# juno181/Ex4DGS

Measured on AMD Instinct MI355X. Metric: fwd+bwd ms/frame @1M Gaussians 1352x1014; achieved HBM GB/s vs peak, lower is better.
Workload: dtype f32; 1 GPU; cfg3: 1.0M static+dynamic (K=35), 1352x1014; P=1000000, HW=1370928, sh_degree=3, step=GaussianRasterizer forward + backward on a resident frame, parallelism=frame-sharded x1

## Files before the change

### ex4dgs_amd/csrc/ex4d_api.hip

```cpp
#include "ex4d_internal.h"
#include <atomic>
#include <cstdarg>
#include <cstdio>
#include <cstdlib>
#include <cstring>
#include <mutex>

namespace {

std::atomic<bool> g_prof_on{false};
std::atomic<int> g_bwd_variant{4};
std::atomic<int> g_tile_ids{0};
std::atomic<int> g_tile_rows{1};
std::atomic<int> g_depth_msd{3};
struct DepthSortWatch {
    std::mutex mu;
    uint32_t *word = nullptr;
    bool tried = false;
    std::atomic<int> hold{0}, backoff{64}, trips{0};
    uint32_t *get()
    {
        std::lock_guard<std::mutex> lock(mu);
        if (!tried) {
            tried = true;
            if (hipHostMalloc((void **)&word, 64, hipHostMallocPortable) != hipSuccess) { (void)hipGetLastError(); word = nullptr; }
            else memset(word, 0, 64);
        }
        return word;
    }
    void reset()
    {
        std::lock_guard<std::mutex> lock(mu);
        hold.store(0); backoff.store(64); trips.store(0);
        if (word) __atomic_store_n(word, 0u, __ATOMIC_RELAXED);
// ... 429 lines not shown
    const float *shs, const float *colors_precomp, const float *scales, const float *rotations,
    const float *cov3D_precomp, const float *viewmatrix, const float *projmatrix, const float *campos,
    const float *subpixel_offset, const float *out_depth, const float *out_acc,
    const void *geom_buffer, const void *binning_buffer, const void *img_buffer,
    const float *dL_dout_color, const float *dL_dout_depth, const float *dL_dout_flow, const float *dL_dout_acc,
    float *dL_dmeans2D, float *dL_dcolors, float *dL_dopacity, float *dL_dmeans3D, float *dL_dcov3D, float *dL_dsh,
    float *dL_dscales, float *dL_drotations, float *dL_ddir, void *bwd_scratch, void *stream_)
{
    g_err[0] = 0;
    hipStream_t stream = (hipStream_t)stream_;
    if (!prm) return fail(EX4D_ERR_ARG, "null params");
    const int P = prm->P, W = prm->W, H = prm->H;
    if (P <= 0 || W <= 0 || H <= 0) return fail(EX4D_ERR_ARG, "P, W, H must be positive (P == 0 is handled by the caller)");
    if (!geom_buffer || !binning_buffer || !img_buffer || !bwd_scratch) return fail(EX4D_ERR_ARG, "null state buffer");
    if ((size_t)P * 64 > 0xFFFFFFFFull) return fail(EX4D_ERR_ARG, "more than 2^26 Gaussians: the accumulator rows are addressed with 32-bit byte offsets");
    if (!dL_dmeans2D || !dL_dopacity || !dL_dmeans3D || !dL_dscales || !dL_drotations || !dL_ddir || (prm->M > 0 && !dL_dsh && !(gsplit.rest[0] || gsplit.rest[1])))
        return fail(EX4D_ERR_ARG, "null gradient output");
    GeomState g = carve_geom((void *)geom_buffer, P, nullptr, nullptr);
    BinState b = carve_binning((void *)binning_buffer, (uint32_t)num_rendered, W, H, nullptr, nullptr);
    ImgState im = carve_img((void *)img_buffer, W, H, nullptr, nullptr);
    float *acc16 = (float *)bwd_scratch;

    const int variant = g_bwd_variant.load(std::memory_order_relaxed);
    g_prof.begin(1, stream);
    HIP_TRY(ex4d_launch_zero(acc16, (size_t)P * 16 * sizeof(float), stream));
    MARK(1, "zero_accumulators");
    if (num_rendered > 0)
        STAGE(ex4d_launch_composite_bwd(*prm, im.ranges, b.point_list, subpixel_offset, background, g.records,
                                        out_depth, out_acc, im.final_T, im.n_contrib,
                                        dL_dout_color, dL_dout_depth, dL_dout_flow, dL_dout_acc, acc16, b.qlist, b.qcount, variant, stream), prm, stream);
    MARK(1, "composite_bwd");
    const float *cov3D_ptr = cov3D_precomp;
    STAGE(ex4d_launch_preprocess_bwd(*prm, means3D, radii, shs, scales, rotations, cov3D_ptr, viewmatrix, projmatrix, campos, g, acc16,
                                     dL_dmeans2D, dL_dcolors, dL_dopacity, dL_dmeans3D, dL_dcov3D, dL_dsh, dL_dscales, dL_drotations, dL_ddir,
                                     split, gsplit, stream), prm, stream);
    MARK(1, "preprocess_bwd");
    return EX4D_OK;
}

static const ShSplit kNoSplit = { { nullptr, nullptr }, { nullptr, nullptr }, 0 };
static const ShSplitGrad kNoSplitGrad = { { nullptr, nullptr }, { nullptr, nullptr }, 0 };

int ex4d_forward(
    const Ex4dParams *prm,
    const float *background, const float *means3D, const float *dir3D, const float *shs, const float *colors_precomp,
    const float *opacities, const float *scales, const float *rotations, const float *cov3D_precomp,
    const float *viewmatrix, const float *projmatrix, const float *campos, const float *subpixel_offset,
    ex4d_alloc_fn geom_alloc, void *geom_user, ex4d_alloc_fn binning_alloc, void *binning_user,
    ex4d_alloc_fn img_alloc, void *img_user,
    float *out_color, int32_t *radii, float *out_depth, float *out_acc, float *out_flow, int32_t *out_idx,
    void *stream_, int32_t *num_rendered)
{
    return forward_impl(prm, kNoSplit, background, means3D, dir3D, shs, colors_precomp, opacities, scales, rotations, cov3D_precomp,
                        viewmatrix, projmatrix, campos, subpixel_offset, geom_alloc, geom_user, binning_alloc, binning_user,
                        img_alloc, img_user, out_color, radii, out_depth, out_acc, out_flow, out_idx, stream_, num_rendered);
}

static bool split_ok(const Ex4dParams *prm, const float *const dc[2], const float *const rest[2], int n_static)
// ... 49 lines not shown
    float *dL_dmeans2D, float *dL_dcolors, float *dL_dopacity, float *dL_dmeans3D, float *dL_dcov3D, const Ex4dSplitSHGrad *dL_dsh,
    float *dL_dscales, float *dL_drotations, float *dL_ddir, void *bwd_scratch, void *stream_)
{
    g_err[0] = 0;
    if (!shs || !dL_dsh || !split_ok(prm, shs->dc, shs->rest, shs->n_static) || dL_dsh->n_static != shs->n_static ||
        !split_ok(prm, (const float *const *)dL_dsh->dc, (const float *const *)dL_dsh->rest, dL_dsh->n_static))
        return fail(EX4D_ERR_ARG, "split SH: null tensor, n_static outside [0, P] or mismatching gradient split");
    if (prm->M != 16) return fail(EX4D_ERR_ARG, "split SH needs M == 16 (dc [n,1,3] + rest [n,15,3])");
    const ShSplit sp = { { shs->dc[0], shs->dc[1] }, { shs->rest[0], shs->rest[1] }, shs->n_static };
    const ShSplitGrad gsp = { { dL_dsh->dc[0], dL_dsh->dc[1] }, { dL_dsh->rest[0], dL_dsh->rest[1] }, dL_dsh->n_static };
    return backward_impl(prm, sp, gsp, num_rendered, background, means3D, radii, nullptr, nullptr, scales, rotations,
                         cov3D_precomp, viewmatrix, projmatrix, campos, subpixel_offset, out_depth, out_acc, geom_buffer, binning_buffer,
                         img_buffer, dL_dout_color, dL_dout_depth, dL_dout_flow, dL_dout_acc, dL_dmeans2D, dL_dcolors, dL_dopacity,
                         dL_dmeans3D, dL_dcov3D, nullptr, dL_dscales, dL_drotations, dL_ddir, bwd_scratch, stream_);
}

int ex4d_set_option(const char *name, int value)
{
    if (name && !strcmp(name, "composite_bwd_variant") && (value == 4 || value == 8)) { g_bwd_variant.store(value); return EX4D_OK; }
    if (name && !strcmp(name, "composite_fwd_asm") && (value == 0 || value == 1)) { ex4d_set_fwd_asm(value); return EX4D_OK; }
    if (name && !strcmp(name, "binning_tile_ids") && (value == 0 || value == 1)) { g_tile_ids.store(value); return EX4D_OK; }
    if (name && !strcmp(name, "composite_clamp_always") && (value == 0 || value == 1)) { ex4d_set_clamp_always(value); return EX4D_OK; }
    if (name && !strcmp(name, "composite_bwd_pairs") && (value == 0 || value == 1)) { ex4d_set_bwd_pairs(value); return EX4D_OK; }
    if (name && !strcmp(name, "tile_sort_rows") && (value == 0 || value == 1)) { g_tile_rows.store(value); return EX4D_OK; }
    if (name && !strcmp(name, "rank_lds_atomics") && value >= -1 && value <= 1) { ex4d_set_rank_lds(value); return EX4D_OK; }
    if (name && !strcmp(name, "rows_probe")) { ex4d_set_rows_probe(value); return EX4D_OK; }
    if (name && !strcmp(name, "preprocess_sh_predicate") && (value == 0 || value == 1)) { ex4d_set_preprocess_tune(value); return EX4D_OK; }
    if (name && !strcmp(name, "geom_debug_arrays") && (value == 0 || value == 1)) { g_geom_debug.store(value); return EX4D_OK; }
    if (name && !strcmp(name, "preprocess_fast_path") && (value == 0 || value == 1)) { ex4d_set_preprocess_fast(value); return EX4D_OK; }
    if (name && !strcmp(name, "depth_sort_msd") && value >= 0 && value <= 3) { g_depth_msd.store(value); g_depth_watch.reset(); return EX4D_OK; }
    if (name && !strcmp(name, "depth_sort_local_cap") && value >= 0 && value <= 8192) { g_depth_local_cap.store(value); return EX4D_OK; }
    if (name && !strcmp(name, "readback_side_stream") && (value == 0 || value == 1)) { g_readback_side.store(value); return EX4D_OK; }
    if (name && !strcmp(name, "depth_sort_msd_bits") && (value == 0 || value == EX4D_DLS_MSD_BITS - 1 || value == EX4D_DLS_MSD_BITS)) { g_depth_msd_bits.store(value); return EX4D_OK; }
    if (name && !strcmp(name, "depth_sort_local_threads") && (value == 0 || value == 256 || value == 512)) { g_depth_local_threads.store(value); return EX4D_OK; }
    return fail(EX4D_ERR_ARG, "unknown option or value out of range");
}

int ex4d_debug_bwd_stats(unsigned long long *out8, int reset) { return ex4d_bwd_stats(out8, 8, reset) == hipSuccess ? EX4D_OK : EX4D_ERR_HIP; }
int ex4d_debug_rows_prof(unsigned long long *out8, int reset) { return ex4d_rows_prof(out8, reset) == hipSuccess ? EX4D_OK : EX4D_ERR_HIP; }
int ex4d_debug_bwd_stats16(unsigned long long *out16, int reset) { return ex4d_bwd_stats(out16, 16, reset) == hipSuccess ? EX4D_OK : EX4D_ERR_HIP; }

int ex4d_get_option(const char *name)
{
    if (name && !strcmp(name, "composite_bwd_variant")) return g_bwd_variant.load();
    if (name && !strcmp(name, "composite_fwd_asm")) return ex4d_get_fwd_asm();
    if (name && !strcmp(name, "binning_tile_ids")) return g_tile_ids.load();
    if (name && !strcmp(name, "composite_clamp_always")) return ex4d_get_clamp_always();
    if (name && !strcmp(name, "composite_bwd_pairs")) return ex4d_get_bwd_pairs();
    if (name && !strcmp(name, "tile_sort_rows")) return g_tile_rows.load();
    if (name && !strcmp(name, "rank_lds_atomics")) return ex4d_get_rank_lds();
    if (name && !strcmp(name, "rank_lds_atomics_in_use")) return ex4d_rank_lds_in_use();
    if (name && !strcmp(name, "preprocess_sh_predicate")) return ex4d_get_preprocess_tune();
    if (name && !strcmp(name, "geom_debug_arrays")) return g_geom_debug.load();
    if (name && !strcmp(name, "preprocess_fast_path")) return ex4d_get_preprocess_fast();
    if (name && !strcmp(name, "depth_sort_msd")) return g_depth_msd.load();
    if (name && !strcmp(name, "depth_sort_hold")) return g_depth_watch.hold.load();
    if (name && !strcmp(name, "depth_sort_trips")) return g_depth_watch.trips.load();
    if (name && !strcmp(name, "depth_sort_local_cap")) return g_depth_local_cap.load();
    if (name && !strcmp(name, "readback_side_stream")) return g_readback_side.load();
    if (name && !strcmp(name, "depth_sort_msd_bits")) return g_depth_msd_bits.load();
    if (name && !strcmp(name, "depth_sort_local_threads")) return g_depth_local_threads.load();
    return -1;
}

void ex4d_profile_enable(int on) { g_prof_on.store(on != 0); }

int ex4d_profile_read(int which, float *ms, const char **names, int max_stages)
{
    std::lock_guard<std::mutex> lock(g_prof.mu);
    if (which < 0 || which > 1 || !g_prof.created) return 0;
    const int n = g_prof.n[which] < max_stages ? g_prof.n[which] : max_stages;
// ... 23 lines not shown
```

### ex4dgs_amd/csrc/ex4d_composite.hip

```cpp
#include "ex4d_internal.h"
#include <hip/amd_detail/amd_hip_unsafe_atomics.h>
#include <atomic>

namespace {

__device__ __forceinline__ void wave_lds_sync()
{
    __builtin_amdgcn_fence(__ATOMIC_RELEASE, "wavefront");
    __builtin_amdgcn_wave_barrier();
    __builtin_amdgcn_fence(__ATOMIC_ACQUIRE, "wavefront");
}

typedef unsigned long long lanemask;
#define LANES(cmp) __builtin_amdgcn_ballot_w64(cmp)
__device__ __forceinline__ float select_f(lanemask m, float if_set, float if_clear)
{
    float r;
    asm("s_nop 1\n\tv_cndmask_b32_e64 %0, %1, %2, %3" : "=v"(r) : "v"(if_clear), "v"(if_set), "s"(m));
    return r;
}
__device__ __forceinline__ int select_i(lanemask m, int if_set, int if_clear)
{
    int r;
    asm("s_nop 1\n\tv_cndmask_b32_e64 %0, %1, %2, %3" : "=v"(r) : "v"(if_clear), "v"(if_set), "s"(m));
// ... 757 lines not shown
    }
    wave_lds_sync();
    {
        float v[13];
        const float Se = S2.x, So = S2.y, Ye = Y2.x, Yo = Y2.y;
        v[0] = dxe * Se + dxo * So;
        v[1] = Ye + Yo;
        v[3] = (dxe * dxe) * Se + (dxo * dxo) * So;
        v[4] = dxe * Ye + dxo * Yo;
        v[0] *= w; v[1] *= w; v[3] *= w; v[4] *= w;
        v[5] = w * (M5.x + M5.y);
        v[2] = v2.x + v2.y; v[6] = Se + So; v[7] = c7.x + c7.y; v[8] = c8.x + c8.y; v[9] = c9.x + c9.y;
        v[10] = c10.x + c10.y; v[11] = c11.x + c11.y; v[12] = c12.x + c12.y;
        {
            const float m0 = v[0], m1 = v[1];
            v[0] = (2.f * ap) * m0 + bp * m1;
            v[1] = (2.f * cp) * m1 + bp * m0;
            v[2] *= flagf;
        }
        bwd_batch_finish<NOLAST>(L, nvalid, acc16, v, __float_as_uint(g1.w), n, g);
    }
}

template <int WPB, bool STATS>
__global__ __launch_bounds__(64 * WPB, 4) void composite_bwd_scan_kernel(
    int W, int H, int gx, int num_tiles,
    const uint2 *__restrict__ ranges, const uint32_t *__restrict__ point_list,
    const float *__restrict__ subpixel_offset, const float *__restrict__ bg,
    const float4 *__restrict__ records,
    const float *__restrict__ depth_acc, const float *__restrict__ weight_acc, float min_depth,
    const float *__restrict__ final_Ts, const uint32_t *__restrict__ n_contrib,
    const float *__restrict__ dL_dpixels, const float *__restrict__ dL_ddepths,
    const float *__restrict__ dL_dflows, const float *__restrict__ dL_daccs,
    float *__restrict__ acc16, const uint32_t *__restrict__ qlist, const uint32_t *__restrict__ qcount, int pairs_on)
{
    constexpr int RING = BWD_RING;
    __shared__ BwdLdsT<RING> lds[WPB];
    int tile, quad;
    tile_of_block(num_tiles, tile, quad);
    if (tile >= num_tiles) return;
    const int wave = (WPB == 4) ? (threadIdx.x >> 6) : 0, lane = threadIdx.x & 63;
    BwdLdsT<RING> &L = lds[wave];
    const PixelGeom p = pixel_of_lane(tile, quad, gx, W, H, subpixel_offset);
    const uint2 range = ranges[tile];
    const size_t HW = (size_t)H * W;
    const uint32_t last_contributor = p.inside ? n_contrib[p.pix_id] : 0u;
    const uint32_t deepest = wave_max_u32(last_contributor);
    if (deepest == 0) return;
    const uint32_t min_last = wave_min_u32(last_contributor);

    const float T_final = p.inside ? final_Ts[p.pix_id] : 0.f;
    const float acc = p.inside ? weight_acc[p.pix_id] : 0.f;
    const float final_depth = p.inside ? depth_acc[p.pix_id] : 0.f;
    float gdepth = 0.f, gflow0 = 0.f, gflow1 = 0.f, gflow2 = 0.f, gacc = 0.f, gp0 = 0.f, gp1 = 0.f, gp2 = 0.f;
    if (p.inside) {
        if (dL_ddepths) gdepth = dL_ddepths[p.pix_id];
        if (dL_dpixels) { gp0 = dL_dpixels[p.pix_id]; gp1 = dL_dpixels[HW + p.pix_id]; gp2 = dL_dpixels[2 * HW + p.pix_id]; }
        if (acc > 0.0f) {
            gdepth /= acc;
            if (dL_dflows) { gflow0 = dL_dflows[p.pix_id] / acc; gflow1 = dL_dflows[HW + p.pix_id] / acc; gflow2 = dL_dflows[2 * HW + p.pix_id] / acc; }
// ... 100 lines not shown

hipError_t ex4d_launch_composite_fwd(const Ex4dParams &prm, const uint2 *ranges, const uint32_t *point_list,
    const float *subpixel_offset, const float4 *records, const float *bg, float *final_T, uint32_t *n_contrib,
    float *out_color, float *out_depth, float *out_acc, float *out_flow, int32_t *out_idx, uint32_t *qlist, uint32_t *qcount,
    bool has_flow, hipStream_t stream)
{
    const int gx = (prm.W + EX4D_TILE - 1) / EX4D_TILE, gy = (prm.H + EX4D_TILE - 1) / EX4D_TILE;
    const int T = gx * gy;
    const int slots = 8 * ((T + 7) / 8);
#define FWD_LAUNCH(FLOW) hipLaunchKernelGGL((composite_fwd_kernel<FLOW, ASM>), dim3(4 * slots), dim3(64), 0, stream, \
        prm.W, prm.H, gx, T, ranges, point_list, subpixel_offset, records, bg, \
        prm.max_depth, final_T, n_contrib, out_color, out_depth, out_acc, out_flow, out_idx, qlist, qcount, g_alpha_clamp_always.load(std::memory_order_relaxed))
    if (has_flow) { constexpr bool ASM = false; FWD_LAUNCH(true); }
    else if (g_fwd_asm.load(std::memory_order_relaxed)) { constexpr bool ASM = true; FWD_LAUNCH(false); }
    else { constexpr bool ASM = false; FWD_LAUNCH(false); }
#undef FWD_LAUNCH
    return hipGetLastError();
}

hipError_t ex4d_launch_composite_bwd(const Ex4dParams &prm, const uint2 *ranges, const uint32_t *point_list,
    const float *subpixel_offset, const float *bg, const float4 *records, const float *out_depth, const float *out_acc,
    const float *final_T, const uint32_t *n_contrib, const float *dL_dpix, const float *dL_ddepth,
    const float *dL_dflow, const float *dL_dacc, float *acc16, const uint32_t *qlist, const uint32_t *qcount,
    int variant, hipStream_t stream)
{
    const int gx = (prm.W + EX4D_TILE - 1) / EX4D_TILE, gy = (prm.H + EX4D_TILE - 1) / EX4D_TILE;
    const int T = gx * gy;
    const int Tpad = 8 * ((T + 7) / 8);
#define BWD_ARGS prm.W, prm.H, gx, T, ranges, point_list, subpixel_offset, bg, records, out_depth, out_acc, prm.min_depth, \
                 final_T, n_contrib, dL_dpix, dL_ddepth, dL_dflow, dL_dacc, acc16
    if (variant == 8) hipLaunchKernelGGL((composite_bwd_scan_kernel<1, true>), dim3(4 * Tpad), dim3(64), 0, stream, BWD_ARGS, qlist, qcount, 0);
    else hipLaunchKernelGGL((composite_bwd_scan_kernel<1, false>), dim3(4 * Tpad), dim3(64), 0, stream, BWD_ARGS, qlist, qcount, g_bwd_pairs.load(std::memory_order_relaxed));
#undef BWD_ARGS
    return hipGetLastError();
}
```

### ex4dgs_amd/csrc/ex4d_internal.h

```cpp
#pragma once
#include <hip/hip_runtime.h>
#include <stdint.h>
#include <stddef.h>
#include "../../include/ex4d_rasterizer.h"
#include "../../include/ex4d_attributes.h"

#define EX4D_ALIGN 256

static inline size_t ex4d_align_up(size_t x) { return (x + (EX4D_ALIGN - 1)) & ~(size_t)(EX4D_ALIGN - 1); }

#define EX4D_RECORD_FLOATS 16
#define EX4D_DLS_MSD_BITS 10
#define EX4D_CHUNK_FLOW 0x80000000u
#define EX4D_CHUNK_FILTERED 0x40000000u
#define EX4D_DSUMS_MARK 0x44535553u

struct GeomState {
    float4 *records;
    float *cov3D;
    uint8_t *clamped;
    uint32_t *tiles_touched;
    uint2 *rects;
    uint2 *sorted_rects;
    uint32_t *rects4;
// ... 31 lines not shown
#define SCAN_CHUNK 2048

static inline uint32_t rs_num_blocks(uint32_t n) { return (n + RS_CHUNK - 1) / RS_CHUNK; }
struct Ex4dTsBlock { uint32_t start, count, bucket, fb_first, fb_next, bucket_start; };
static inline uint32_t ex4d_tile_sort_pass_b_blocks(uint32_t R, int nbuckets) { return rs_num_blocks(R) + (uint32_t)nbuckets + 1u; }

struct ShSplit { const float *dc[2]; const float *rest[2]; int n_static; };
struct ShSplitGrad { float *dc[2]; float *rest[2]; int n_static; };

hipError_t ex4d_launch_preprocess_fwd(const Ex4dParams &prm, const float *means3D, const float *dir3D, const float *scales,
    const float *rotations, const float *opacities, const float *shs, const float *cov3D_precomp,
    const float *colors_precomp, const float *viewmatrix, const float *projmatrix, const float *campos,
    int32_t *radii, GeomState g, uint32_t *prefilter_violation, ShSplit split,
    uint32_t *depth_keys, uint32_t *depth_vals, uint32_t depth_key_base, uint32_t depth_key_invisible, uint32_t *rects4, hipStream_t stream,
    uint32_t *key_range_slots = nullptr, bool global_flags = true);

hipError_t ex4d_launch_mark_visible(int P, const float *means3D, const float *viewmatrix, const float *projmatrix,
    float min_depth, float max_depth, uint8_t *present, hipStream_t stream);

hipError_t ex4d_launch_preprocess_bwd(const Ex4dParams &prm, const float *means3D, const int32_t *radii,
    const float *shs, const float *scales, const float *rotations, const float *cov3D_ptr,
    const float *viewmatrix, const float *projmatrix, const float *campos, GeomState g, const float *acc16,
    float *dL_dmeans2D, float *dL_dcolors, float *dL_dopacity, float *dL_dmeans3D, float *dL_dcov3D, float *dL_dsh,
    float *dL_dscales, float *dL_drotations, float *dL_ddir, ShSplit split, ShSplitGrad gsplit, hipStream_t stream);

hipError_t ex4d_radix_sort_pairs(uint32_t *keys_a, uint32_t *vals_a, uint32_t *keys_b, uint32_t *vals_b,
    uint32_t n, int end_bit, uint32_t *hist, bool *result_in_a, hipStream_t stream, const uint32_t *n_dev = nullptr, bool iota_values = false,
    const uint32_t *gather_in = nullptr, uint32_t *gather_out = nullptr, uint2 *zero_ranges = nullptr, int num_ranges = 0);
size_t ex4d_radix_hist_words(uint32_t n);
int ex4d_radix_passes(uint32_t n, int end_bit);

bool ex4d_tile_sort_msd_applies(int P, int tile_bits);
size_t ex4d_tile_sort_hist_words(uint32_t R, int tile_bits);
hipError_t ex4d_tile_sort_msd(const uint32_t *keys, const uint32_t *vals, uint32_t *packed, uint32_t *point_list, uint32_t *tile_ids_out,
    uint32_t R, int tile_bits, uint32_t *hist, uint2 *ranges, hipStream_t stream, const uint32_t *n_dev = nullptr);

bool ex4d_tile_sort_rows_applies(int P, int gx, int gy);
size_t ex4d_tile_sort_rows_geom_words(uint32_t P);
size_t ex4d_tile_sort_rows_hist_words(uint32_t R);
void ex4d_set_rows_probe(int v);
hipError_t ex4d_rows_prof(unsigned long long *out8, int reset);
hipError_t ex4d_tile_sort_rows(int P, int gx, int gy, const uint32_t *order, const uint32_t *r4, const uint2 *r8, uint32_t *words,
    uint32_t *point_list, uint32_t *tile_ids_out, uint32_t cap, uint32_t S, uint32_t *histA, uint32_t *histB, uint2 *ranges, uint32_t *frame_total, hipStream_t stream);

hipError_t ex4d_launch_scan_tiles(int P, const uint2 *rects, const uint32_t *rects4, const uint32_t *order, uint2 *sorted_rects, uint32_t *sorted_offsets,
    uint32_t *block_sums, int T, uint2 *ranges, uint32_t *frame_total, hipStream_t stream);
hipError_t ex4d_launch_duplicate(int P, int W, int H, const uint32_t *order, const uint32_t *sorted_offsets,
// ... 12 lines not shown
int ex4d_depth_sort_msd_bits(uint32_t n, int key_bits);
void ex4d_set_rank_lds(int v);
int ex4d_get_rank_lds();
int ex4d_rank_lds_in_use();
hipError_t ex4d_prepare_rank_lds(hipStream_t stream);
hipError_t ex4d_launch_zero(void *ptr, size_t bytes, hipStream_t stream);
hipError_t ex4d_launch_tile_ranges(uint32_t R, int T, const uint32_t *tile_ids, uint2 *ranges, hipStream_t stream, const uint32_t *n_dev = nullptr);

void ex4d_set_preprocess_tune(int v);
int ex4d_get_preprocess_tune();
void ex4d_set_preprocess_fast(int v);
int ex4d_get_preprocess_fast();
void ex4d_set_fwd_asm(int on);
int ex4d_get_fwd_asm();
void ex4d_set_clamp_always(int on);
int ex4d_get_clamp_always();
void ex4d_set_bwd_pairs(int on);
int ex4d_get_bwd_pairs();
hipError_t ex4d_launch_composite_fwd(const Ex4dParams &prm, const uint2 *ranges, const uint32_t *point_list,
    const float *subpixel_offset, const float4 *records, const float *bg, float *final_T, uint32_t *n_contrib,
    float *out_color, float *out_depth, float *out_acc, float *out_flow, int32_t *out_idx, uint32_t *qlist, uint32_t *qcount,
    bool has_flow, hipStream_t stream);

hipError_t ex4d_launch_composite_bwd(const Ex4dParams &prm, const uint2 *ranges, const uint32_t *point_list,
    const float *subpixel_offset, const float *bg, const float4 *records, const float *out_depth, const float *out_acc,
    const float *final_T, const uint32_t *n_contrib, const float *dL_dpix, const float *dL_ddepth,
    const float *dL_dflow, const float *dL_dacc, float *acc16, const uint32_t *qlist, const uint32_t *qcount,
    int variant, hipStream_t stream);

hipError_t ex4d_bwd_stats(unsigned long long *out, int count, int reset);
```

### ex4dgs_amd/csrc/ex4d_preprocess.hip

```cpp
#include "ex4d_internal.h"
#include <atomic>
#include <cstdlib>
#include <cstdlib>

namespace {

__constant__ float kSH_C0 = 0.28209479177387814f;
__constant__ float kSH_C1 = 0.4886025119029199f;
__constant__ float kSH_C2[5] = { 1.0925484305920792f, -1.0925484305920792f, 0.31539156525252005f,
                                 -1.0925484305920792f, 0.5462742152960396f };
__constant__ float kSH_C3[7] = { -0.5900435899266435f, 2.890611442640554f, -0.4570457994644658f, 0.3731763325901154f,
                                 -0.4570457994644658f, 1.445305721320277f, -0.5900435899266435f };

struct Mat3 { float m[3][3]; };

__device__ __forceinline__ Mat3 mul(const Mat3 &a, const Mat3 &b)
{
    Mat3 o;
#pragma unroll
    for (int c = 0; c < 3; c++)
#pragma unroll
        for (int r = 0; r < 3; r++)
            o.m[c][r] = a.m[0][r] * b.m[c][0] + a.m[1][r] * b.m[c][1] + a.m[2][r] * b.m[c][2];
    return o;
// ... 225 lines not shown
    const int part = all_dynamic ? 1 : 0;
    const size_t r0 = (size_t)(wave_first - (part ? sp.n_static : 0));
    return ((((uintptr_t)(sp.rest[part] + r0 * 45)) | ((uintptr_t)(sp.dc[part] + r0 * 3))) & 15) == 0;
}
__device__ __forceinline__ void wave_load_sh_split_half(const ShSplit &sp, int wave_first, float *lds, int lane, int h, uint64_t need)
{
    const int part = wave_first >= sp.n_static ? 1 : 0;
    const size_t r0 = (size_t)(wave_first - (part ? sp.n_static : 0)) + 32 * h;
    const float4 *rest = reinterpret_cast<const float4 *>(sp.rest[part] + r0 * 45);
    const uint32_t need_h = (uint32_t)(need >> (32 * h));
    float4 t[6];
#pragma unroll
    for (int i = 0; i < 6; i++) {
        const int q = i * 64 + lane;
        const int r_lo = (4 * q) / 45, r_hi = (4 * q + 3) / 45;
        const bool want = q < 360 && (((need_h >> r_lo) | (need_h >> (r_hi & 31))) & 1u);
        t[i] = want ? rest[q] : make_float4(0.f, 0.f, 0.f, 0.f);
    }
#pragma unroll
    for (int i = 0; i < 6; i++) { const int q = i * 64 + lane; if (q < 360) reinterpret_cast<float4 *>(lds)[q] = t[i]; }
    wave_sync_lds();
}

__device__ __forceinline__ void wave_store_sh_split_half(const ShSplitGrad &sp, int first, const float *lds, int lane)
{
    wave_sync_lds();
    const int part = first >= sp.n_static ? 1 : 0;
    const size_t r0 = (size_t)(first - (part ? sp.n_static : 0));
    float4 *rest = reinterpret_cast<float4 *>(sp.rest[part] + r0 * 45), *dc = reinterpret_cast<float4 *>(sp.dc[part] + r0 * 3);
#pragma unroll
    for (int i = 0; i < 6; i++) { const int q = i * 64 + lane; if (q < 360) rest[q] = reinterpret_cast<const float4 *>(lds)[q]; }
    if (lane < 24) dc[lane] = reinterpret_cast<const float4 *>(lds + SH_HALF_DC_OFFSET)[lane];
}

__device__ __forceinline__ void wave_store_sh_half(float *__restrict__ dst_half, const float *lds, int nrows, int lane)
{
    wave_sync_lds();
    float4 *dst = reinterpret_cast<float4 *>(dst_half);
#pragma unroll
    for (int it = 0; it < 6; it++) {
        const int q = it * 64 + lane;
        const int g = q / 12, v = q - 12 * g;
        if (g < nrows) dst[q] = *reinterpret_cast<const float4 *>(lds + g * SH_ROW + 4 * v);
    }
}





__device__ __forceinline__ void sh_direction_sums(const float *sh, int D, float x, float y, float z,
                                                  float (&dRGBdx)[3], float (&dRGBdy)[3], float (&dRGBdz)[3])
{
#define SHK(k) sh[3 * (k) + ch]
    if (D > 0) {
#pragma unroll
        for (int ch = 0; ch < 3; ch++) {
            dRGBdx[ch] = -kSH_C1 * SHK(3);
            dRGBdy[ch] = -kSH_C1 * SHK(1);
            dRGBdz[ch] = kSH_C1 * SHK(2);
        }
        if (D > 1) {
            const float xx = x * x, yy = y * y, zz = z * z, xy = x * y, yz = y * z, xz = x * z;
#pragma unroll
            for (int ch = 0; ch < 3; ch++) {
                dRGBdx[ch] += kSH_C2[0] * y * SHK(4) + kSH_C2[2] * 2.f * -x * SHK(6) + kSH_C2[3] * z * SHK(7) + kSH_C2[4] * 2.f * x * SHK(8);
// ... 310 lines not shown
        depth_keys[idx] = depth_key;
        if (depth_vals) depth_vals[idx] = (uint32_t)idx;
    }
    uint32_t wave_sum = out_tiles, wave_seg = visible ? (rect.y >> 16) : 0u;
#pragma unroll
    for (int o = 32; o > 0; o >>= 1) { wave_sum += __shfl_xor(wave_sum, o, 64); wave_seg += __shfl_xor(wave_seg, o, 64); }
    if (lane == 0) reinterpret_cast<uint2 *>(total_instances)[wc] = make_uint2(wave_sum, wave_seg | (chunk_flow ? EX4D_CHUNK_FLOW : 0u) | (chunk_filtered ? EX4D_CHUNK_FILTERED : 0u));
}

__global__ __launch_bounds__(256) void mark_visible_kernel(int P, const float *__restrict__ means3D,
    const float *__restrict__ viewmatrix, const float *__restrict__ projmatrix, float min_depth, float max_depth,
    uint8_t *__restrict__ present)
{
    const int idx = blockIdx.x * 256 + threadIdx.x;
    if (idx >= P) return;
    float vm[16], pm[16];
#pragma unroll
    for (int i = 0; i < 16; i++) { vm[i] = viewmatrix[i]; pm[i] = projmatrix[i]; }
    const float3 p = make_float3(means3D[3 * (size_t)idx], means3D[3 * (size_t)idx + 1], means3D[3 * (size_t)idx + 2]);
    float3 pv; float nx, ny;
    present[idx] = frustum_test(p, vm, pm, min_depth, max_depth, pv, nx, ny) ? 1 : 0;
}

template <bool DSUMS>
__global__ __launch_bounds__(256) void preprocess_bwd_kernel(
    int P, int D, int M,
    const float *__restrict__ means3D, const int32_t *__restrict__ radii, const float *__restrict__ shs,
    const uint8_t *__restrict__ clamped, const float *__restrict__ scales, const float *__restrict__ rotations,
    float scale_modifier, const float *__restrict__ cov3Ds, const float *__restrict__ viewmatrix,
    const float *__restrict__ projmatrix, const float *__restrict__ campos,
    int W, int H, float fx, float fy, float tanx, float tany, float kernel_size,
    const float *__restrict__ acc16, const float4 *__restrict__ records,
    float *__restrict__ dL_dmeans2D, float *__restrict__ dL_dcolors, float *__restrict__ dL_dopacity,
    float *__restrict__ dL_dmeans3D, float *__restrict__ dL_dcov3D, float *__restrict__ dL_dsh,
    float *__restrict__ dL_dscales, float *__restrict__ dL_drotations, float *__restrict__ dL_ddir, const ShSplit sp, const ShSplitGrad gsp,
    const float *__restrict__ sh_dsums, const uint32_t *__restrict__ frame_flags)
{
    __shared__ __attribute__((aligned(16))) float sh_lds[4 * SH_HALF_FLOATS];
    const int idx = blockIdx.x * 256 + threadIdx.x;
    const int lane = threadIdx.x & 63, wave = threadIdx.x >> 6;
    const bool in_range = idx < P;
    const bool split = sp.rest[0] != nullptr || sp.rest[1] != nullptr;
    const bool staged = (shs != nullptr || split) && (M == 16);
    float *lds_row_base = sh_lds + wave * SH_HALF_FLOATS;
    const bool dsums_ok = !DSUMS || frame_flags[3] == EX4D_DSUMS_MARK;
    const int wave_first = blockIdx.x * 256 + wave * 64;
    const int wave_rows = (P - wave_first) < 64 ? (P - wave_first) : 64;
// ... 13 lines not shown
            for (int i = 0; i < 6; i++) in_cov[i] = cov3Ds[6 * (size_t)idx + i];
        }
        if (scales) {
            in_q = reinterpret_cast<const float4 *>(rotations)[idx];
#pragma unroll
            for (int i = 0; i < 3; i++) in_s[i] = scales[3 * (size_t)idx + i];
        }
        if (shs || split) in_clamped = clamped[idx];
    }
    const bool visible = in_range && (in_radius > 0);
    float g_mean2D[3] = { 0, 0, 0 }, g_color[3] = { 0, 0, 0 }, g_dir[3] = { 0, 0, 0 }, g_opacity = 0;
    float g_mean3D[3] = { 0, 0, 0 }, g_cov[6] = { 0, 0, 0, 0, 0, 0 }, g_scale[3] = { 0, 0, 0 }, g_rot[4] = { 0, 0, 0, 0 };
    float3 sh_dir = make_float3(0.f, 0.f, 0.f), sh_dir_orig = make_float3(0.f, 0.f, 0.f);
    float sh_dRGB[3] = { 0.f, 0.f, 0.f }, sh_j[3] = { 0.f, 0.f, 0.f };
    if (visible && (shs || split)) {
        const float3 dir_orig = make_float3(in_mean[0] - campos[0], in_mean[1] - campos[1], in_mean[2] - campos[2]);
        const float len = sqrtf(dir_orig.x * dir_orig.x + dir_orig.y * dir_orig.y + dir_orig.z * dir_orig.z);
        sh_dir = make_float3(dir_orig.x / len, dir_orig.y / len, dir_orig.z / len);
        sh_dir_orig = dir_orig;
        const float gc[3] = { in_r1.w, in_r2.x, in_r2.y };
#pragma unroll
        for (int ch = 0; ch < 3; ch++) sh_dRGB[ch] = gc[ch] * (((in_clamped >> ch) & 1) ? 0.f : 1.f);
    }
    if (shs || split) {
        float dRGBdx[3] = { 0, 0, 0 }, dRGBdy[3] = { 0, 0, 0 }, dRGBdz[3] = { 0, 0, 0 };
        const int r = lane & 31;
        const uint64_t need_rows = __ballot(visible);
        if (DSUMS) {
            if (visible) {
                const float *o = sh_dsums + 9 * (size_t)idx;
#pragma unroll
                for (int ch = 0; ch < 3; ch++) { dRGBdx[ch] = o[ch]; dRGBdy[ch] = o[3 + ch]; dRGBdz[ch] = o[6 + ch]; }
                if (!dsums_ok) { const float nan = __int_as_float(0x7fc00000); for (int ch = 0; ch < 3; ch++) dRGBdx[ch] = dRGBdy[ch] = dRGBdz[ch] = nan; }
            }
        } else if (staged && prefetched) {
#pragma unroll
            for (int h = 0; h < 2; h++) {
                if (split) wave_load_sh_split_half(sp, wave_first, lds_row_base, lane, h, need_rows);
                else wave_load_sh_half(shs + (size_t)wave_first * 48, lds_row_base, wave_rows, ((D + 1) * (D + 1) * 3 + 3) / 4, lane, h, need_rows);
                if (visible && (lane >> 5) == h) {
                    if (split) sh_direction_sums(lds_row_base + r * 45 - 3, D, sh_dir.x, sh_dir.y, sh_dir.z, dRGBdx, dRGBdy, dRGBdz);
                    else sh_direction_sums(lds_row_base + r * SH_ROW, D, sh_dir.x, sh_dir.y, sh_dir.z, dRGBdx, dRGBdy, dRGBdz);
                }
                wave_sync_lds();
            }
        } else if (visible) {
// ... 89 lines not shown
#pragma unroll
                for (int rI = 0; rI < 3; rI++) M2.m[cI][rI] = Mx.m[cI][rI] * 2.0f;
            Mat3 dM = mul(M2, dSigma);
            Mat3 Rt = transpose(R);
            Mat3 dMt = transpose(dM);
#pragma unroll
            for (int k = 0; k < 3; k++)
                g_scale[k] = Rt.m[k][0] * dMt.m[k][0] + Rt.m[k][1] * dMt.m[k][1] + Rt.m[k][2] * dMt.m[k][2];
#pragma unroll
            for (int k = 0; k < 3; k++)
#pragma unroll
                for (int rI = 0; rI < 3; rI++) dMt.m[k][rI] *= s[k];
#define DM(i, j) dMt.m[i][j]
            g_rot[0] = 2 * z * (DM(0,1) - DM(1,0)) + 2 * y * (DM(2,0) - DM(0,2)) + 2 * x * (DM(1,2) - DM(2,1));
            g_rot[1] = 2 * y * (DM(1,0) + DM(0,1)) + 2 * z * (DM(2,0) + DM(0,2)) + 2 * r * (DM(1,2) - DM(2,1)) - 4 * x * (DM(2,2) + DM(1,1));
            g_rot[2] = 2 * x * (DM(1,0) + DM(0,1)) + 2 * r * (DM(2,0) - DM(0,2)) + 2 * z * (DM(1,2) + DM(2,1)) - 4 * y * (DM(2,2) + DM(0,0));
            g_rot[3] = 2 * r * (DM(0,1) - DM(1,0)) + 2 * x * (DM(2,0) + DM(0,2)) + 2 * y * (DM(1,2) + DM(2,1)) - 4 * z * (DM(1,1) + DM(0,0));
#undef DM
        }
    }
    float g_sh[16][3];
#pragma unroll
    for (int k = 0; k < 16; k++) g_sh[k][0] = g_sh[k][1] = g_sh[k][2] = 0.f;
    if (visible && (shs || split)) {
        const float x = sh_dir.x, y = sh_dir.y, z = sh_dir.z;
        const float *dRGB = sh_dRGB;
#define DSH(k, coefexpr) { const float c_ = (coefexpr); g_sh[k][0] = c_ * dRGB[0]; g_sh[k][1] = c_ * dRGB[1]; g_sh[k][2] = c_ * dRGB[2]; }
        DSH(0, kSH_C0)
        if (D > 0) {
            DSH(1, -kSH_C1 * y)
            DSH(2, kSH_C1 * z)
            DSH(3, -kSH_C1 * x)
            if (D > 1) {
                const float xx = x * x, yy = y * y, zz = z * z, xy = x * y, yz = y * z, xz = x * z;
                DSH(4, kSH_C2[0] * xy)
                DSH(5, kSH_C2[1] * yz)
                DSH(6, kSH_C2[2] * (2.f * zz - xx - yy))
                DSH(7, kSH_C2[3] * xz)
                DSH(8, kSH_C2[4] * (xx - yy))
                if (D > 2) {
                    DSH(9, kSH_C3[0] * y * (3.f * xx - yy))
                    DSH(10, kSH_C3[1] * xy * z)
                    DSH(11, kSH_C3[2] * y * (4.f * zz - xx - yy))
                    DSH(12, kSH_C3[3] * z * (2.f * zz - 3.f * xx - 3.f * yy))
                    DSH(13, kSH_C3[4] * x * (4.f * zz - xx - yy))
                    DSH(14, kSH_C3[5] * z * (xx - yy))
                    DSH(15, kSH_C3[6] * x * (xx - 3.f * yy))
                }
            }
        }
#undef DSH
    }
    bool store_staged = prefetched;
    if (split && prefetched) {
        const int part = wave_first >= gsp.n_static ? 1 : 0;
        const size_t r0 = (size_t)(wave_first - (part ? gsp.n_static : 0));
        store_staged = ((((uintptr_t)(gsp.rest[part] + r0 * 45)) | ((uintptr_t)(gsp.dc[part] + r0 * 3))) & 15) == 0;
    }
    if (M == 16 && split && !store_staged) {
        if (in_range) {
            const int part = idx >= gsp.n_static;
            const size_t row = (size_t)(idx - (part ? gsp.n_static : 0));
            float *dc = gsp.dc[part] + row * 3, *rest = gsp.rest[part] + row * 45;
#pragma unroll
            for (int ch = 0; ch < 3; ch++) dc[ch] = g_sh[0][ch];
#pragma unroll
            for (int k = 1; k < 16; k++)
#pragma unroll
                for (int ch = 0; ch < 3; ch++) rest[3 * (k - 1) + ch] = g_sh[k][ch];
        }
    } else if (M == 16) {
#pragma unroll
        for (int h = 0; h < 2; h++) {
            wave_sync_lds();
            if ((lane >> 5) == h) {
                const int r = lane & 31;
                if (split) {
#pragma unroll
                    for (int ch = 0; ch < 3; ch++) lds_row_base[SH_HALF_DC_OFFSET + r * 3 + ch] = g_sh[0][ch];
#pragma unroll
                    for (int k = 1; k < 16; k++)
#pragma unroll
                        for (int ch = 0; ch < 3; ch++) lds_row_base[r * 45 + 3 * (k - 1) + ch] = g_sh[k][ch];
                } else {
                    float4 *row = reinterpret_cast<float4 *>(lds_row_base + r * SH_ROW);
#pragma unroll
                    for (int v = 0; v < 12; v++) {
                        float t[4];
#pragma unroll
                        for (int e = 0; e < 4; e++) { const int f = 4 * v + e; t[e] = g_sh[f / 3][f % 3]; }
                        row[v] = make_float4(t[0], t[1], t[2], t[3]);
                    }
                }
            }
            const int first = wave_first + 32 * h;
            const int nrows_sh = (P - first) < 32 ? (P - first) : 32;
            if (split) wave_store_sh_split_half(gsp, first, lds_row_base, lane);
            else wave_store_sh_half(dL_dsh + (size_t)first * 48, lds_row_base, nrows_sh, lane);
        }
        wave_sync_lds();
    }
    {
        const int nrows = (P - wave_first) < 64 ? (P - wave_first) : 64;
        wave_store_rows<3>(dL_dmeans2D + 3 * (size_t)wave_first, g_mean2D, lds_row_base, nrows, lane);
        if (dL_dcolors) wave_store_rows<3>(dL_dcolors + 3 * (size_t)wave_first, g_color, lds_row_base, nrows, lane);
        wave_store_rows<3>(dL_dmeans3D + 3 * (size_t)wave_first, g_mean3D, lds_row_base, nrows, lane);
        wave_store_rows<3>(dL_dscales + 3 * (size_t)wave_first, g_scale, lds_row_base, nrows, lane);
        wave_store_rows<3>(dL_ddir + 3 * (size_t)wave_first, g_dir, lds_row_base, nrows, lane);
        if (dL_dcov3D) wave_store_rows<6>(dL_dcov3D + 6 * (size_t)wave_first, g_cov, lds_row_base, nrows, lane);
    }
    if (!in_range) return;
    dL_dopacity[idx] = g_opacity;
    reinterpret_cast<float4 *>(dL_drotations)[idx] = make_float4(g_rot[0], g_rot[1], g_rot[2], g_rot[3]);
    if (M != 16) {
#pragma unroll
        for (int k = 0; k < 16; k++)
            if (k < M) {
#pragma unroll
                for (int ch = 0; ch < 3; ch++) dL_dsh[((size_t)idx * M + k) * 3 + ch] = g_sh[k][ch];
            }
        for (int k = 16; k < M; k++)
            for (int ch = 0; ch < 3; ch++) dL_dsh[((size_t)idx * M + k) * 3 + ch] = 0.f;
    }
}

}

static int preprocess_option_default() { const char *e = getenv("EX4D_PREPROCESS_SH_PREDICATE"); return e ? (atoi(e) != 0) : 1; }
static std::atomic<int> g_preprocess_fast{1};
void ex4d_set_preprocess_fast(int v) { g_preprocess_fast.store(v); }
int ex4d_get_preprocess_fast() { return g_preprocess_fast.load(); }
static std::atomic<int> g_preprocess_tune{preprocess_option_default()};
void ex4d_set_preprocess_tune(int v) { g_preprocess_tune.store(v != 0); }
int ex4d_get_preprocess_tune() { return g_preprocess_tune.load(); }

hipError_t ex4d_launch_preprocess_fwd(const Ex4dParams &prm, const float *means3D, const float *dir3D, const float *scales,
    const float *rotations, const float *opacities, const float *shs, const float *cov3D_precomp,
// ... 11 lines not shown
        viewmatrix, projmatrix, campos, prm.W, prm.H, prm.tanfovx, prm.tanfovy, fx, fy, prm.kernel_size, \
        prm.min_depth, prm.max_depth, prm.prefiltered, prefilter_violation, \
        radii, g.records, g.cov3D, g.clamped, g.tiles_touched, g.rects, depth_keys, depth_vals, depth_key_base, depth_key_invisible, g.block_totals, split, \
        (prm.prepare_backward && (shs != nullptr || is_split)) ? g.sh_dsums : (float *)nullptr, \
        g_preprocess_tune.load(std::memory_order_relaxed), rects4, key_range_slots, global_flags ? 1 : 0
    if (fast) hipLaunchKernelGGL(preprocess_fwd_kernel<true>, dim3((prm.P + 255) / 256), dim3(256), 0, stream, PF_ARGS);
    else hipLaunchKernelGGL(preprocess_fwd_kernel<false>, dim3((prm.P + 255) / 256), dim3(256), 0, stream, PF_ARGS);
#undef PF_ARGS
    return hipGetLastError();
}

hipError_t ex4d_launch_mark_visible(int P, const float *means3D, const float *viewmatrix, const float *projmatrix,
    float min_depth, float max_depth, uint8_t *present, hipStream_t stream)
{
    hipLaunchKernelGGL(mark_visible_kernel, dim3((P + 255) / 256), dim3(256), 0, stream,
        P, means3D, viewmatrix, projmatrix, min_depth, max_depth, present);
    return hipGetLastError();
}

hipError_t ex4d_launch_preprocess_bwd(const Ex4dParams &prm, const float *means3D, const int32_t *radii,
    const float *shs, const float *scales, const float *rotations, const float *cov3D_ptr,
    const float *viewmatrix, const float *projmatrix, const float *campos, GeomState g, const float *acc16,
    float *dL_dmeans2D, float *dL_dcolors, float *dL_dopacity, float *dL_dmeans3D, float *dL_dcov3D, float *dL_dsh,
    float *dL_dscales, float *dL_drotations, float *dL_ddir, ShSplit split, ShSplitGrad gsplit, hipStream_t stream)
{
    const float fy = prm.H / (2.0f * prm.tanfovy);
    const float fx = prm.W / (2.0f * prm.tanfovx);
#define PB_ARGS prm.P, prm.D, prm.M, means3D, radii, shs, g.clamped, scales, rotations, prm.scale_modifier, cov3D_ptr, \
        viewmatrix, projmatrix, campos, prm.W, prm.H, fx, fy, prm.tanfovx, prm.tanfovy, prm.kernel_size, acc16, g.records, \
        dL_dmeans2D, dL_dcolors, dL_dopacity, dL_dmeans3D, dL_dcov3D, dL_dsh, dL_dscales, dL_drotations, dL_ddir, split, gsplit
    const bool has_sh = shs != nullptr || split.rest[0] != nullptr || split.rest[1] != nullptr;
    if (prm.prepare_backward && has_sh)
        hipLaunchKernelGGL(preprocess_bwd_kernel<true>, dim3((prm.P + 255) / 256), dim3(256), 0, stream, PB_ARGS, (const float *)g.sh_dsums, (const uint32_t *)g.total);
    else
        hipLaunchKernelGGL(preprocess_bwd_kernel<false>, dim3((prm.P + 255) / 256), dim3(256), 0, stream, PB_ARGS, (const float *)nullptr, (const uint32_t *)g.total);
#undef PB_ARGS
    return hipGetLastError();
}
```

Baseline: 0.6721 ms/frame.

## Zero SH gradients inside composite backward and store only touched SH rows

The SH-gradient buffers are zero-filled by the composite backward kernel: each block clears a share of them with float4 stores. The preprocess backward kernel then writes SH gradient rows only for Gaussians whose colour gradient is nonzero, using a per-wave ballot mask. The goal is to cut HBM write traffic for the large SH gradient tensor (48 floats per Gaussian) when many Gaussians are invisible or receive no gradient. The cost is an extra fill pass folded into the composite kernel's grid, which may lengthen that kernel or compete with it for bandwidth. It also adds new template variants and a dependency on kernel ordering for correctness.

```diff
diff --git a/ex4dgs_amd/csrc/ex4d_api.hip b/ex4dgs_amd/csrc/ex4d_api.hip
--- a/ex4dgs_amd/csrc/ex4d_api.hip
+++ b/ex4dgs_amd/csrc/ex4d_api.hip
@@ -10,6 +10,7 @@
 
 std::atomic<bool> g_prof_on{false};
 std::atomic<int> g_bwd_variant{4};
+std::atomic<int> g_bwd_sparse_sh{1};
 std::atomic<int> g_tile_ids{0};
 std::atomic<int> g_tile_rows{1};
 std::atomic<int> g_depth_msd{3};
@@ -485,18 +486,32 @@
     float *acc16 = (float *)bwd_scratch;
 
     const int variant = g_bwd_variant.load(std::memory_order_relaxed);
+    const bool is_split = gsplit.rest[0] || gsplit.rest[1];
+    const bool sparse_sh = g_bwd_sparse_sh.load(std::memory_order_relaxed) != 0 && num_rendered > 0 && variant != 8 && prm->M > 0 &&
+                           ((shs != nullptr && dL_dsh != nullptr) || is_split);
+    Ex4dZeroSpans fill = {};
+    if (sparse_sh && is_split) {
+        const size_t n[2] = { (size_t)gsplit.n_static, (size_t)P - (size_t)gsplit.n_static };
+        for (int part = 0; part < 2; part++) {
+            if (n[part] == 0) continue;
+            fill.ptr[fill.n] = gsplit.dc[part];   fill.bytes[fill.n++] = n[part] * 3 * sizeof(float);
+            fill.ptr[fill.n] = gsplit.rest[part]; fill.bytes[fill.n++] = n[part] * 45 * sizeof(float);
+        }
+    } else if (sparse_sh) {
+        fill.ptr[0] = dL_dsh; fill.bytes[0] = (size_t)P * (size_t)prm->M * 3 * sizeof(float); fill.n = 1;
+    }
     g_prof.begin(1, stream);
     HIP_TRY(ex4d_launch_zero(acc16, (size_t)P * 16 * sizeof(float), stream));
     MARK(1, "zero_accumulators");
     if (num_rendered > 0)
         STAGE(ex4d_launch_composite_bwd(*prm, im.ranges, b.point_list, subpixel_offset, background, g.records,
                                         out_depth, out_acc, im.final_T, im.n_contrib,
-                                        dL_dout_color, dL_dout_depth, dL_dout_flow, dL_dout_acc, acc16, b.qlist, b.qcount, variant, stream), prm, stream);
+                                        dL_dout_color, dL_dout_depth, dL_dout_flow, dL_dout_acc, acc16, b.qlist, b.qcount, variant, stream, fill), prm, stream);
     MARK(1, "composite_bwd");
     const float *cov3D_ptr = cov3D_precomp;
     STAGE(ex4d_launch_preprocess_bwd(*prm, means3D, radii, shs, scales, rotations, cov3D_ptr, viewmatrix, projmatrix, campos, g, acc16,
                                      dL_dmeans2D, dL_dcolors, dL_dopacity, dL_dmeans3D, dL_dcov3D, dL_dsh, dL_dscales, dL_drotations, dL_ddir,
-                                     split, gsplit, stream), prm, stream);
+                                     split, gsplit, stream, sparse_sh), prm, stream);
     MARK(1, "preprocess_bwd");
     return EX4D_OK;
 }
@@ -592,6 +607,7 @@
     if (name && !strcmp(name, "binning_tile_ids") && (value == 0 || value == 1)) { g_tile_ids.store(value); return EX4D_OK; }
     if (name && !strcmp(name, "composite_clamp_always") && (value == 0 || value == 1)) { ex4d_set_clamp_always(value); return EX4D_OK; }
     if (name && !strcmp(name, "composite_bwd_pairs") && (value == 0 || value == 1)) { ex4d_set_bwd_pairs(value); return EX4D_OK; }
+    if (name && !strcmp(name, "backward_sparse_sh") && (value == 0 || value == 1)) { g_bwd_sparse_sh.store(value); return EX4D_OK; }
     if (name && !strcmp(name, "tile_sort_rows") && (value == 0 || value == 1)) { g_tile_rows.store(value); return EX4D_OK; }
     if (name && !strcmp(name, "rank_lds_atomics") && value >= -1 && value <= 1) { ex4d_set_rank_lds(value); return EX4D_OK; }
     if (name && !strcmp(name, "rows_probe")) { ex4d_set_rows_probe(value); return EX4D_OK; }
@@ -617,6 +633,7 @@
     if (name && !strcmp(name, "binning_tile_ids")) return g_tile_ids.load();
     if (name && !strcmp(name, "composite_clamp_always")) return ex4d_get_clamp_always();
     if (name && !strcmp(name, "composite_bwd_pairs")) return ex4d_get_bwd_pairs();
+    if (name && !strcmp(name, "backward_sparse_sh")) return g_bwd_sparse_sh.load();
     if (name && !strcmp(name, "tile_sort_rows")) return g_tile_rows.load();
     if (name && !strcmp(name, "rank_lds_atomics")) return ex4d_get_rank_lds();
     if (name && !strcmp(name, "rank_lds_atomics_in_use")) return ex4d_rank_lds_in_use();
diff --git a/ex4dgs_amd/csrc/ex4d_composite.hip b/ex4dgs_amd/csrc/ex4d_composite.hip
--- a/ex4dgs_amd/csrc/ex4d_composite.hip
+++ b/ex4dgs_amd/csrc/ex4d_composite.hip
@@ -803,6 +803,29 @@
     }
 }
 
+__device__ __forceinline__ void zero_fill_share(const Ex4dZeroSpans &z, uint32_t block, uint32_t nblocks, int lane)
+{
+#pragma unroll
+    for (int s = 0; s < 4; s++) {
+        if (s >= z.n) break;
+        char *const p = static_cast<char *>(z.ptr[s]);
+        const size_t bytes = (size_t)z.bytes[s];
+        size_t head = (size_t)((16u - (uint32_t)((uintptr_t)p & 15u)) & 15u);
+        if (head > bytes) head = bytes;
+        const size_t nvec = (bytes - head) >> 4;
+        const size_t share = (nvec + nblocks - 1) / nblocks;
+        const size_t lo = (size_t)block * share < nvec ? (size_t)block * share : nvec;
+        const size_t hi = lo + share < nvec ? lo + share : nvec;
+        float4 *const body = reinterpret_cast<float4 *>(p + head);
+        for (size_t i = lo + (size_t)lane; i < hi; i += 64) body[i] = make_float4(0.f, 0.f, 0.f, 0.f);
+        if (block == 0) {
+            const size_t tail = bytes - head - (nvec << 4);
+            if ((size_t)lane < head) p[lane] = 0;
+            if ((size_t)lane < tail) p[head + (nvec << 4) + (size_t)lane] = 0;
+        }
+    }
+}
+
 template <int WPB, bool STATS>
 __global__ __launch_bounds__(64 * WPB, 4) void composite_bwd_scan_kernel(
     int W, int H, int gx, int num_tiles,
@@ -813,10 +836,11 @@
     const float *__restrict__ final_Ts, const uint32_t *__restrict__ n_contrib,
     const float *__restrict__ dL_dpixels, const float *__restrict__ dL_ddepths,
     const float *__restrict__ dL_dflows, const float *__restrict__ dL_daccs,
-    float *__restrict__ acc16, const uint32_t *__restrict__ qlist, const uint32_t *__restrict__ qcount, int pairs_on)
+    float *__restrict__ acc16, const uint32_t *__restrict__ qlist, const uint32_t *__restrict__ qcount, int pairs_on, const Ex4dZeroSpans fill)
 {
     constexpr int RING = BWD_RING;
     __shared__ BwdLdsT<RING> lds[WPB];
+    if (!STATS) zero_fill_share(fill, blockIdx.x, gridDim.x, threadIdx.x & 63);
     int tile, quad;
     tile_of_block(num_tiles, tile, quad);
     if (tile >= num_tiles) return;
@@ -963,15 +987,16 @@
     const float *subpixel_offset, const float *bg, const float4 *records, const float *out_depth, const float *out_acc,
     const float *final_T, const uint32_t *n_contrib, const float *dL_dpix, const float *dL_ddepth,
     const float *dL_dflow, const float *dL_dacc, float *acc16, const uint32_t *qlist, const uint32_t *qcount,
-    int variant, hipStream_t stream)
+    int variant, hipStream_t stream, const Ex4dZeroSpans &fill)
 {
     const int gx = (prm.W + EX4D_TILE - 1) / EX4D_TILE, gy = (prm.H + EX4D_TILE - 1) / EX4D_TILE;
     const int T = gx * gy;
     const int Tpad = 8 * ((T + 7) / 8);
+    if (variant == 8 && fill.n != 0) return hipErrorInvalidValue;
 #define BWD_ARGS prm.W, prm.H, gx, T, ranges, point_list, subpixel_offset, bg, records, out_depth, out_acc, prm.min_depth, \
                  final_T, n_contrib, dL_dpix, dL_ddepth, dL_dflow, dL_dacc, acc16
-    if (variant == 8) hipLaunchKernelGGL((composite_bwd_scan_kernel<1, true>), dim3(4 * Tpad), dim3(64), 0, stream, BWD_ARGS, qlist, qcount, 0);
-    else hipLaunchKernelGGL((composite_bwd_scan_kernel<1, false>), dim3(4 * Tpad), dim3(64), 0, stream, BWD_ARGS, qlist, qcount, g_bwd_pairs.load(std::memory_order_relaxed));
+    if (variant == 8) hipLaunchKernelGGL((composite_bwd_scan_kernel<1, true>), dim3(4 * Tpad), dim3(64), 0, stream, BWD_ARGS, qlist, qcount, 0, fill);
+    else hipLaunchKernelGGL((composite_bwd_scan_kernel<1, false>), dim3(4 * Tpad), dim3(64), 0, stream, BWD_ARGS, qlist, qcount, g_bwd_pairs.load(std::memory_order_relaxed), fill);
 #undef BWD_ARGS
     return hipGetLastError();
 }
diff --git a/ex4dgs_amd/csrc/ex4d_internal.h b/ex4dgs_amd/csrc/ex4d_internal.h
--- a/ex4dgs_amd/csrc/ex4d_internal.h
+++ b/ex4dgs_amd/csrc/ex4d_internal.h
@@ -77,7 +77,8 @@
     const float *shs, const float *scales, const float *rotations, const float *cov3D_ptr,
     const float *viewmatrix, const float *projmatrix, const float *campos, GeomState g, const float *acc16,
     float *dL_dmeans2D, float *dL_dcolors, float *dL_dopacity, float *dL_dmeans3D, float *dL_dcov3D, float *dL_dsh,
-    float *dL_dscales, float *dL_drotations, float *dL_ddir, ShSplit split, ShSplitGrad gsplit, hipStream_t stream);
+    float *dL_dscales, float *dL_drotations, float *dL_ddir, ShSplit split, ShSplitGrad gsplit, hipStream_t stream,
+    bool sparse_sh = false);
 
 hipError_t ex4d_radix_sort_pairs(uint32_t *keys_a, uint32_t *vals_a, uint32_t *keys_b, uint32_t *vals_b,
     uint32_t n, int end_bit, uint32_t *hist, bool *result_in_a, hipStream_t stream, const uint32_t *n_dev = nullptr, bool iota_values = false,
@@ -136,10 +137,11 @@
     float *out_color, float *out_depth, float *out_acc, float *out_flow, int32_t *out_idx, uint32_t *qlist, uint32_t *qcount,
     bool has_flow, hipStream_t stream);
 
+struct Ex4dZeroSpans { void *ptr[4]; unsigned long long bytes[4]; int n; };
 hipError_t ex4d_launch_composite_bwd(const Ex4dParams &prm, const uint2 *ranges, const uint32_t *point_list,
     const float *subpixel_offset, const float *bg, const float4 *records, const float *out_depth, const float *out_acc,
     const float *final_T, const uint32_t *n_contrib, const float *dL_dpix, const float *dL_ddepth,
     const float *dL_dflow, const float *dL_dacc, float *acc16, const uint32_t *qlist, const uint32_t *qcount,
-    int variant, hipStream_t stream);
+    int variant, hipStream_t stream, const Ex4dZeroSpans &fill = Ex4dZeroSpans{});
 
 hipError_t ex4d_bwd_stats(unsigned long long *out, int count, int reset);
diff --git a/ex4dgs_amd/csrc/ex4d_preprocess.hip b/ex4dgs_amd/csrc/ex4d_preprocess.hip
--- a/ex4dgs_amd/csrc/ex4d_preprocess.hip
+++ b/ex4dgs_amd/csrc/ex4d_preprocess.hip
@@ -271,18 +271,29 @@
     wave_sync_lds();
 }
 
-__device__ __forceinline__ void wave_store_sh_split_half(const ShSplitGrad &sp, int first, const float *lds, int lane)
+template <bool SPARSE>
+__device__ __forceinline__ void wave_store_sh_split_half(const ShSplitGrad &sp, int first, const float *lds, int lane, uint32_t rows)
 {
     wave_sync_lds();
     const int part = first >= sp.n_static ? 1 : 0;
     const size_t r0 = (size_t)(first - (part ? sp.n_static : 0));
     float4 *rest = reinterpret_cast<float4 *>(sp.rest[part] + r0 * 45), *dc = reinterpret_cast<float4 *>(sp.dc[part] + r0 * 3);
 #pragma unroll
-    for (int i = 0; i < 6; i++) { const int q = i * 64 + lane; if (q < 360) rest[q] = reinterpret_cast<const float4 *>(lds)[q]; }
-    if (lane < 24) dc[lane] = reinterpret_cast<const float4 *>(lds + SH_HALF_DC_OFFSET)[lane];
-}
-
-__device__ __forceinline__ void wave_store_sh_half(float *__restrict__ dst_half, const float *lds, int nrows, int lane)
+    for (int i = 0; i < 6; i++) {
+        const int q = i * 64 + lane;
+        const int r_lo = (4 * q) / 45, r_hi = (4 * q + 3) / 45;
+        const bool want = !SPARSE || (((rows >> (r_lo & 31)) | (rows >> (r_hi & 31))) & 1u);
+        if (q < 360 && want) rest[q] = reinterpret_cast<const float4 *>(lds)[q];
+    }
+    {
+        const int r_lo = (4 * lane) / 3, r_hi = (4 * lane + 3) / 3;
+        const bool want = !SPARSE || (((rows >> (r_lo & 31)) | (rows >> (r_hi & 31))) & 1u);
+        if (lane < 24 && want) dc[lane] = reinterpret_cast<const float4 *>(lds + SH_HALF_DC_OFFSET)[lane];
+    }
+}
+
+template <bool SPARSE>
+__device__ __forceinline__ void wave_store_sh_half(float *__restrict__ dst_half, const float *lds, int nrows, int lane, uint32_t rows)
 {
     wave_sync_lds();
     float4 *dst = reinterpret_cast<float4 *>(dst_half);
@@ -290,7 +301,7 @@
     for (int it = 0; it < 6; it++) {
         const int q = it * 64 + lane;
         const int g = q / 12, v = q - 12 * g;
-        if (g < nrows) dst[q] = *reinterpret_cast<const float4 *>(lds + g * SH_ROW + 4 * v);
+        if (g < nrows && (!SPARSE || ((rows >> g) & 1u))) dst[q] = *reinterpret_cast<const float4 *>(lds + g * SH_ROW + 4 * v);
     }
 }
 
@@ -647,7 +658,7 @@
     present[idx] = frustum_test(p, vm, pm, min_depth, max_depth, pv, nx, ny) ? 1 : 0;
 }
 
-template <bool DSUMS>
+template <bool DSUMS, bool SPARSE>
 __global__ __launch_bounds__(256) void preprocess_bwd_kernel(
     int P, int D, int M,
     const float *__restrict__ means3D, const int32_t *__restrict__ radii, const float *__restrict__ shs,
@@ -707,6 +718,8 @@
 #pragma unroll
         for (int ch = 0; ch < 3; ch++) sh_dRGB[ch] = gc[ch] * (((in_clamped >> ch) & 1) ? 0.f : 1.f);
     }
+    const bool sh_touched = !SPARSE || (visible && (sh_dRGB[0] != 0.f || sh_dRGB[1] != 0.f || sh_dRGB[2] != 0.f));
+    const uint64_t touched_rows = SPARSE ? __ballot(sh_touched) : ~0ull;
     if (shs || split) {
         float dRGBdx[3] = { 0, 0, 0 }, dRGBdy[3] = { 0, 0, 0 }, dRGBdz[3] = { 0, 0, 0 };
         const int r = lane & 31;
@@ -842,7 +855,7 @@
     float g_sh[16][3];
 #pragma unroll
     for (int k = 0; k < 16; k++) g_sh[k][0] = g_sh[k][1] = g_sh[k][2] = 0.f;
-    if (visible && (shs || split)) {
+    if (visible && (shs || split) && sh_touched) {
         const float x = sh_dir.x, y = sh_dir.y, z = sh_dir.z;
         const float *dRGB = sh_dRGB;
 #define DSH(k, coefexpr) { const float c_ = (coefexpr); g_sh[k][0] = c_ * dRGB[0]; g_sh[k][1] = c_ * dRGB[1]; g_sh[k][2] = c_ * dRGB[2]; }
@@ -878,7 +891,7 @@
         store_staged = ((((uintptr_t)(gsp.rest[part] + r0 * 45)) | ((uintptr_t)(gsp.dc[part] + r0 * 3))) & 15) == 0;
     }
     if (M == 16 && split && !store_staged) {
-        if (in_range) {
+        if (in_range && sh_touched) {
             const int part = idx >= gsp.n_static;
             const size_t row = (size_t)(idx - (part ? gsp.n_static : 0));
             float *dc = gsp.dc[part] + row * 3, *rest = gsp.rest[part] + row * 45;
@@ -892,8 +905,10 @@
     } else if (M == 16) {
 #pragma unroll
         for (int h = 0; h < 2; h++) {
+            const uint32_t rows_h = (uint32_t)(touched_rows >> (32 * h));
+            if (SPARSE && rows_h == 0u) continue;
             wave_sync_lds();
-            if ((lane >> 5) == h) {
+            if ((lane >> 5) == h && (!SPARSE || split || sh_touched)) {
                 const int r = lane & 31;
                 if (split) {
 #pragma unroll
@@ -915,8 +930,8 @@
             }
             const int first = wave_first + 32 * h;
             const int nrows_sh = (P - first) < 32 ? (P - first) : 32;
-            if (split) wave_store_sh_split_half(gsp, first, lds_row_base, lane);
-            else wave_store_sh_half(dL_dsh + (size_t)first * 48, lds_row_base, nrows_sh, lane);
+            if (split) wave_store_sh_split_half<SPARSE>(gsp, first, lds_row_base, lane, rows_h);
+            else wave_store_sh_half<SPARSE>(dL_dsh + (size_t)first * 48, lds_row_base, nrows_sh, lane, rows_h);
         }
         wave_sync_lds();
     }
@@ -932,7 +947,7 @@
     if (!in_range) return;
     dL_dopacity[idx] = g_opacity;
     reinterpret_cast<float4 *>(dL_drotations)[idx] = make_float4(g_rot[0], g_rot[1], g_rot[2], g_rot[3]);
-    if (M != 16) {
+    if (M != 16 && sh_touched) {
 #pragma unroll
         for (int k = 0; k < 16; k++)
             if (k < M) {
@@ -990,7 +1005,7 @@
     const float *shs, const float *scales, const float *rotations, const float *cov3D_ptr,
     const float *viewmatrix, const float *projmatrix, const float *campos, GeomState g, const float *acc16,
     float *dL_dmeans2D, float *dL_dcolors, float *dL_dopacity, float *dL_dmeans3D, float *dL_dcov3D, float *dL_dsh,
-    float *dL_dscales, float *dL_drotations, float *dL_ddir, ShSplit split, ShSplitGrad gsplit, hipStream_t stream)
+    float *dL_dscales, float *dL_drotations, float *dL_ddir, ShSplit split, ShSplitGrad gsplit, hipStream_t stream, bool sparse_sh)
 {
     const float fy = prm.H / (2.0f * prm.tanfovy);
     const float fx = prm.W / (2.0f * prm.tanfovx);
@@ -998,10 +1013,11 @@
         viewmatrix, projmatrix, campos, prm.W, prm.H, fx, fy, prm.tanfovx, prm.tanfovy, prm.kernel_size, acc16, g.records, \
         dL_dmeans2D, dL_dcolors, dL_dopacity, dL_dmeans3D, dL_dcov3D, dL_dsh, dL_dscales, dL_drotations, dL_ddir, split, gsplit
     const bool has_sh = shs != nullptr || split.rest[0] != nullptr || split.rest[1] != nullptr;
-    if (prm.prepare_backward && has_sh)
-        hipLaunchKernelGGL(preprocess_bwd_kernel<true>, dim3((prm.P + 255) / 256), dim3(256), 0, stream, PB_ARGS, (const float *)g.sh_dsums, (const uint32_t *)g.total);
-    else
-        hipLaunchKernelGGL(preprocess_bwd_kernel<false>, dim3((prm.P + 255) / 256), dim3(256), 0, stream, PB_ARGS, (const float *)nullptr, (const uint32_t *)g.total);
+    if (sparse_sh && !has_sh) return hipErrorInvalidValue;
+#define PB_LAUNCH(DSUMS, SPARSE, dsums) hipLaunchKernelGGL((preprocess_bwd_kernel<DSUMS, SPARSE>), dim3((prm.P + 255) / 256), dim3(256), 0, stream, PB_ARGS, (const float *)(dsums), (const uint32_t *)g.total)
+    if (prm.prepare_backward && has_sh) { if (sparse_sh) PB_LAUNCH(true, true, g.sh_dsums); else PB_LAUNCH(true, false, g.sh_dsums); }
+    else { if (sparse_sh) PB_LAUNCH(false, true, nullptr); else PB_LAUNCH(false, false, nullptr); }
+#undef PB_LAUNCH
 #undef PB_ARGS
     return hipGetLastError();
 }
```

Result: no change. 0.6739 ms/frame (+0.3%).
